# sparcityeu/SparseBase

Measured on AMD Instinct MI355X. Metric: Mrows/s, RCM reorder + CSR permute, 100M-nnz power-law (RMAT) CSR, higher is better.
Workload: dtype int32

## Files before the change

sparsebase_amd/csrc/sbx_countsort.h:

```cpp
#pragma once
#include "sbx_device.h"
#include "sbx_internal.h"
#include <utility>

namespace sbx_cs {
namespace {

constexpr int ROUNDS = 4;
constexpr int TILE = 256 * ROUNDS;
constexpr int64_t MAX_PAIRS = (int64_t)1 << 20;

template <int BITS>
__device__ __forceinline__ unsigned long long peers_of(unsigned d, bool valid) {
  unsigned long long peers = __ballot(valid);
#pragma unroll
  for (int b = 0; b < BITS; b++) {
    const bool bit = (d >> b) & 1u;
    const unsigned long long m = __ballot(bit);
    peers &= bit ? m : ~m;
  }
  return peers;
}

template <int BITS>
// ... 67 lines not shown
                                                  Emit emit) {
  constexpr int BINS = 1 << BITS, PER = BINS / 256;
  __shared__ unsigned s_scan[8];
  __shared__ unsigned s_wave[4][BINS];
  const int lane = sbx_lane(), wv = sbx_wave_in_block();
  const int64_t j0 = (int64_t)blockIdx.x * TILE + wv * (64 * ROUNDS) + lane;
  unsigned kk[ROUNDS], vv[ROUNDS];
#pragma unroll
  for (int r = 0; r < ROUNDS; r++) {
    const int64_t j = j0 + r * 64;
    kk[r] = key[j < n ? j : n - 1];
    vv[r] = val[j < n ? j : n - 1];
  }
  unsigned tt[PER], oo[PER], tsum = 0;
#pragma unroll
  for (int k = 0; k < PER; k++) {
    tt[k] = total[PER * threadIdx.x + k];
    oo[k] = off[(int64_t)(PER * threadIdx.x + k) * n_tiles + blockIdx.x];
    tsum += tt[k];
  }
#pragma unroll
  for (int w = 0; w < 4; w++)
#pragma unroll
    for (int k = 0; k < PER; k++) s_wave[w][PER * threadIdx.x + k] = 0;
  unsigned tot;
  const unsigned dbase = sbx_block_exclusive_sum<unsigned, 256>(tsum, s_scan, &tot);
  unsigned loc[ROUNDS];
#pragma unroll
  for (int r = 0; r < ROUNDS; r++) {
    const bool valid = j0 + r * 64 < n;
    const unsigned d = (kk[r] >> shift) & mask;
    const unsigned long long peers = peers_of<BITS>(d, valid);
    const unsigned rank = (unsigned)__popcll(peers & sbx_lanemask_lt());
    unsigned first = 0;
    if (valid && rank == 0) first = atomicAdd(&s_wave[wv][d], (unsigned)__popcll(peers));
    first = (unsigned)__shfl((int)first, valid ? (int)__builtin_ctzll(peers) : 0, 64);
    loc[r] = first + rank;
  }
  __syncthreads();
  {
    unsigned before = dbase;
#pragma unroll
    for (int k = 0; k < PER; k++) {
      unsigned run = before + oo[k];
#pragma unroll
      for (int w = 0; w < 4; w++) {
        const unsigned c = s_wave[w][PER * threadIdx.x + k];
        s_wave[w][PER * threadIdx.x + k] = run;
        run += c;
      }
      before += tt[k];
    }
  }
  __syncthreads();
#pragma unroll
  for (int r = 0; r < ROUNDS; r++) {
    if (j0 + r * 64 < n) {
      const unsigned d = (kk[r] >> shift) & mask;
      const unsigned pos = s_wave[wv][d] + loc[r];
      if (last) {
        emit(pos, kk[r], vv[r]);
      } else {
        key_out[pos] = kk[r];
        val_out[pos] = vv[r];
      }
    }
  }
}

static inline size_t scratch_words(int64_t n) { return (size_t)((n + TILE - 1) / TILE) * 512 + 512; }
template <int BITS, typename Emit>
static int digit_pass(sbx_handle_t h, int kid, const uint32_t *ka, const uint32_t *va, uint32_t *kb, uint32_t *vb, int64_t n,
                      int shift, int width, int last, unsigned *scratch, Emit emit) {
  constexpr int BINS = 1 << BITS;
  const int64_t n_tiles = (n + TILE - 1) / TILE;
  unsigned *total = scratch, *cnt = scratch + BINS;
  const unsigned mask = (1u << width) - 1u;
  SBX_KLAUNCH(h, kid, k_cs_count<BITS>, dim3((unsigned)n_tiles), dim3(256), ka, n, n_tiles, shift, mask, cnt);
  SBX_KLAUNCH(h, kid, k_cs_scan, dim3(BINS), dim3(256), cnt, n_tiles, total);
  SBX_KLAUNCH(h, kid, (k_cs_place<BITS, Emit>), dim3((unsigned)n_tiles), dim3(256), ka, va, n, n_tiles, (const unsigned *)cnt,
              (const unsigned *)total, shift, mask, kb, vb, last, emit);
  return SBX_OK;
}
template <typename Emit>
static int sort_emit(sbx_handle_t h, int kid, uint32_t *ka, uint32_t *va, uint32_t *kb, uint32_t *vb, int64_t n, int bits,
                     Emit emit, unsigned *scratch = nullptr) {
  if (!scratch) SBX_TRY(sbx_salloc(h, scratch_words(n), &scratch));
  if (bits < 1) bits = 1;
  const int np = (bits + 8) / 9;
  for (int p = 0, shift = 0; p < np; p++) {
    const int width = (bits - shift + (np - p) - 1) / (np - p);
    const int last = p == np - 1 ? 1 : 0;
    SBX_TRY((digit_pass<9, Emit>(h, kid, ka, va, kb, vb, n, shift, width, last, scratch, emit)));
    std::swap(ka, kb);
    std::swap(va, vb);
    shift += width;
  }
  SBX_LAUNCH_CHECK(h);
  return SBX_OK;
}

}
}
```

sparsebase_amd/csrc/sbx_rcm.hip:

```cpp
#include "sbx_device.h"
#include "sbx_internal.h"
#include "sbx_countsort.h"

#include <utility>
#include <algorithm>
#include <vector>
#include <functional>
#include <string>

namespace {

typedef int32_t I;
#ifdef SBX_RCM_I64
typedef int64_t X;
#define SBX_RCM_IT SBX_I64
#define SBX_RCM_ENTRY sbx_rcm_reorder_x64
#else
typedef int32_t X;
#define SBX_RCM_IT SBX_I32
#define SBX_RCM_ENTRY sbx_rcm_reorder_x32
#endif
constexpr int RCM_SMALL = 64;
constexpr int RCM_MID = 2048;
constexpr int RCM_MID_BATCH = 64;
// ... 974 lines not shown
                                                    RcmDev *__restrict__ dv) {
  int64_t j = (int64_t)blockIdx.x * blockDim.x + threadIdx.x;
  const int64_t stride = (int64_t)gridDim.x * blockDim.x;
  for (; j < nf; j += stride) {
    const uint32_t lo = (uint32_t)key[j];
    const I v = (I)(CM ? dorder[lo] : lo);
    q_level[j] = v;
    if (set_bits) atomicOr(&vbits[v >> 5], 1u << (v & 31));
    if (mark_frontier) {
      if (set_bits) atomicOr(&fbits[v >> 5], 1u << (v & 31));
      lpos[v] = (unsigned)j;
    }
  }
  if (blockIdx.x == 0 && threadIdx.x == 0) {
    dv->nf = 0;
    dv->n_heavy = 0;
    dv->hub_overflow = 0;
    dv->fedges = 0;
  }
}

__global__ __launch_bounds__(256) void k_visited_from_ppos(const unsigned *__restrict__ ppos,
                                                           unsigned long long *__restrict__ vbits64,
                                                           unsigned long long *__restrict__ fbits64, int64_t n) {
  const int64_t wave = ((int64_t)blockIdx.x * blockDim.x + threadIdx.x) >> 6;
  const int64_t nwaves = ((int64_t)gridDim.x * blockDim.x) >> 6;
  const int lane = sbx_lane();
  for (int64_t base = wave * 64; base < n; base += nwaves * 64) {
    const int64_t v = base + lane;
    const bool seen = v < n && ppos[v] != UNSEEN;
    const unsigned long long now = __ballot(seen);
    if (lane == 0) {
      const unsigned long long before = vbits64[base >> 6];
      vbits64[base >> 6] = now;
      if (fbits64) fbits64[base >> 6] = now & ~before;
    }
  }
}

constexpr int RCM_FW_WORDS = 64;
constexpr int RCM_FW_INLINE = 4096;

__global__ __launch_bounds__(256) void k_fresh_words(const unsigned *__restrict__ ppos,
                                                     unsigned long long *__restrict__ vbits64,
                                                     unsigned long long *__restrict__ fbits64,
                                                     unsigned long long *__restrict__ fresh64, int *__restrict__ cnt,
                                                     int *__restrict__ btot, int64_t n) {
  constexpr int WPW = RCM_FW_WORDS / 4;
  __shared__ int s_tot;
  __shared__ unsigned long long s_now[4][WPW];
  if (threadIdx.x == 0) s_tot = 0;
  __syncthreads();
  const int lane = sbx_lane(), wv = threadIdx.x >> 6;
  const int64_t w0 = (int64_t)blockIdx.x * RCM_FW_WORDS + (int64_t)wv * WPW;
  unsigned pv[WPW];
#pragma unroll
  for (int i = 0; i < WPW; i++) {
    const int64_t v = (w0 + i) * 64 + lane;
    pv[i] = v < n ? ppos[v] : UNSEEN;
  }
#pragma unroll
  for (int i = 0; i < WPW; i++) {
    const unsigned long long now = __ballot(pv[i] != UNSEEN);
    if (lane == 0) s_now[wv][i] = now;
  }
  __builtin_amdgcn_wave_barrier();
  int mine = 0;
  if (lane < WPW && (w0 + lane) * 64 < n) {
    const int64_t w = w0 + lane;
    const unsigned long long now = s_now[wv][lane];
    const unsigned long long fresh = now & ~vbits64[w];
    vbits64[w] = now;
    if (fbits64) fbits64[w] = fresh;
    fresh64[w] = fresh;
    mine = __popcll(fresh);
    cnt[w] = mine;
  }
  mine = sbx_wave_sum(mine);
  if (lane == 0 && mine) atomicAdd(&s_tot, mine);
  __syncthreads();
  if (threadIdx.x == 0) btot[blockIdx.x] = s_tot;
}

__global__ __launch_bounds__(256) void k_fresh_words_ranked(const unsigned *__restrict__ ppos,
                                                            const unsigned *__restrict__ vbits,
                                                            const uint32_t *__restrict__ dorder,
                                                            unsigned long long *__restrict__ fresh64,
                                                            int *__restrict__ cnt, int *__restrict__ btot,
                                                            int64_t n_ranked) {
  constexpr int WPW = RCM_FW_WORDS / 4;
  __shared__ int s_tot;
  if (threadIdx.x == 0) s_tot = 0;
  __syncthreads();
  const int lane = sbx_lane(), wv = threadIdx.x >> 6;
  const int64_t w0 = (int64_t)blockIdx.x * RCM_FW_WORDS + (int64_t)wv * WPW;
  uint32_t vv[WPW];
#pragma unroll
  for (int i = 0; i < WPW; i++) {
    const int64_t k = (w0 + i) * 64 + lane;
    vv[i] = dorder[k < n_ranked ? k : n_ranked - 1];
  }
  unsigned pv[WPW], vw[WPW];
#pragma unroll
  for (int i = 0; i < WPW; i++) pv[i] = ppos[vv[i]], vw[i] = vbits[vv[i] >> 5];
  int mine = 0;
#pragma unroll
  for (int i = 0; i < WPW; i++) {
    const int64_t k = (w0 + i) * 64 + lane;
    const bool fresh = k < n_ranked && pv[i] != UNSEEN && !((vw[i] >> (vv[i] & 31)) & 1u);
    const unsigned long long f = __ballot(fresh);
    if (lane == 0 && (w0 + i) * 64 < n_ranked) {
      fresh64[w0 + i] = f;
      cnt[w0 + i] = __popcll(f);
      mine += __popcll(f);
    }
  }
  if (lane == 0 && mine) atomicAdd(&s_tot, mine);
  __syncthreads();
  if (threadIdx.x == 0) btot[blockIdx.x] = s_tot;
}

__global__ __launch_bounds__(256) void k_keys_from_fresh(unsigned long long *__restrict__ fresh64,
                                                         const int *__restrict__ cnt, const int *__restrict__ btot,
                                                         int btot_is_scanned, const unsigned *__restrict__ ppos,
                                                         const uint32_t *__restrict__ dorder,
                                                         uint64_t *__restrict__ key, uint32_t *__restrict__ key32,
                                                         uint32_t *__restrict__ val32, int64_t words,
                                                         RcmDev *__restrict__ dv) {
  constexpr int WPW = RCM_FW_WORDS / 4;
  const int lane = sbx_lane(), wv = threadIdx.x >> 6;
  if (blockIdx.x == 0 && threadIdx.x == 0) reset_level_counters(dv);
  int base = 0;
  if (btot_is_scanned) {
    base = btot[blockIdx.x];
  } else {
    for (int i = lane; i < (int)blockIdx.x; i += 64) base += btot[i];
    base = sbx_wave_sum(base);
  }
  const int64_t wb = (int64_t)blockIdx.x * RCM_FW_WORDS;
  const int c = wb + lane < words ? cnt[wb + lane] : 0;
  const int inc = sbx_wave_inclusive_sum(c);
  const int excl = base + inc - c;
  const bool own = lane >= wv * WPW && lane < (wv + 1) * WPW && wb + lane < words;
  const unsigned long long mine = own ? fresh64[wb + lane] : 0ull;
  if (key32 && mine) fresh64[wb + lane] = 0;
  uint32_t vtx[WPW], low[WPW];
  int at[WPW];
  unsigned long long onmask = 0;
#pragma unroll
  for (int i = 0; i < WPW; i++) {
    const int src = wv * WPW + i;
    const unsigned long long f = __shfl(mine, src, 64);
    const int o = __shfl(excl, src, 64);
    const bool on = (f >> lane) & 1ull;
    low[i] = (uint32_t)((wb + src) * 64 + lane);
    at[i] = o + __popcll(f & sbx_lanemask_lt());
    if (on) onmask |= 1ull << i;
    vtx[i] = (on && dorder) ? dorder[low[i]] : low[i];
  }
  unsigned pp[WPW];
#pragma unroll
  for (int i = 0; i < WPW; i++) pp[i] = ((onmask >> i) & 1ull) ? ppos[vtx[i]] : 0u;
#pragma unroll
  for (int i = 0; i < WPW; i++) {
    if ((onmask >> i) & 1ull) {
      if (key32) {
        key32[at[i]] = pp[i];
        val32[at[i]] = low[i];
      } else {
        key[at[i]] = ((uint64_t)pp[i] << 32) | (uint64_t)low[i];
      }
    }
  }
}

__global__ __launch_bounds__(256) void k_rank_scatter(const I *__restrict__ nf_list, unsigned nf,
                                                      const uint32_t *__restrict__ drank,
                                                      unsigned long long *__restrict__ fresh64) {
  int64_t j = (int64_t)blockIdx.x * blockDim.x + threadIdx.x;
  const int64_t stride = (int64_t)gridDim.x * blockDim.x;
  for (; j < nf; j += stride) {
    const I v = nf_list[j];
    const uint32_t k = drank ? drank[v] : (uint32_t)v;
    atomicOr(&fresh64[k >> 6], 1ull << (k & 63));
  }
}
__global__ __launch_bounds__(64) void k_rank_counts(const unsigned long long *__restrict__ fresh64, int *__restrict__ cnt,
                                                    int *__restrict__ btot, int64_t words) {
  const int64_t w = (int64_t)blockIdx.x * RCM_FW_WORDS + threadIdx.x;
  const int c = w < words ? __popcll(fresh64[w]) : 0;
  if (w < words) cnt[w] = c;
  const int t = sbx_wave_sum(c);
  if (threadIdx.x == 0) btot[blockIdx.x] = t;
}

struct LevelEmit {
  const uint32_t *map;
  I *out;
  unsigned *bits_a, *bits_b, *pos_of;
  __device__ void operator()(unsigned pos, uint32_t, uint32_t val) const {
    const uint32_t v = map ? map[val] : val;
    out[pos] = (I)v;
    if (bits_a) atomicOr(&bits_a[v >> 5], 1u << (v & 31));
    if (bits_b) atomicOr(&bits_b[v >> 5], 1u << (v & 31));
    if (pos_of) pos_of[v] = pos;
  }
};

constexpr int RCM_BR_MAX = 48;
template <bool CM>
__global__ __launch_bounds__(1024) void k_level_sort_small(const I *__restrict__ nf_list, unsigned nf,
                                                           const unsigned *__restrict__ ppos,
                                                           const uint32_t *__restrict__ drank,
                                                           const uint32_t *__restrict__ dorder,
                                                           I *__restrict__ q_level, unsigned *__restrict__ vbits,
                                                           unsigned *__restrict__ fbits, unsigned *__restrict__ lpos,
                                                           int mark_frontier, RcmDev *__restrict__ dv) {
  constexpr int IPT = RCM_LDS_SORT / 1024;
  __shared__ uint64_t s_key[RCM_LDS_SORT];
  __shared__ uint64_t s_tmp[RCM_LDS_SORT];
  __shared__ unsigned s_end[RCM_LDS_SORT];
  __shared__ uint64_t s_mn[16], s_mx[16];
  __shared__ unsigned s_wsum[16], s_big;
  const int lane = sbx_lane(), wv = threadIdx.x >> 6;
  uint64_t mk[IPT];
  uint64_t mn = ~0ull, mx = 0;
#pragma unroll
  for (int i = 0; i < IPT; i++) {
    const unsigned j = threadIdx.x + i * 1024;
    mk[i] = ~0ull;
    if (j < nf) {
      const I v = nf_list[j];
      mk[i] = ((uint64_t)ppos[v] << 32) | (uint64_t)(CM ? drank[v] : (uint32_t)v);
      mn = mk[i] < mn ? mk[i] : mn;
      mx = mk[i] > mx ? mk[i] : mx;
    }
    s_end[j] = 0;
  }
  mn = sbx_wave_min(mn);
  mx = sbx_wave_max(mx);
  if (lane == 0) {
    s_mn[wv] = mn;
    s_mx[wv] = mx;
  }
  if (threadIdx.x == 0) s_big = 0;
  __syncthreads();
#pragma unroll
  for (int i = 0; i < 16; i++) {
    mn = s_mn[i] < mn ? s_mn[i] : mn;
    mx = s_mx[i] > mx ? s_mx[i] : mx;
  }
  const uint64_t range = mx - mn;
  int shift = 0;
  while (shift < 64 && (range >> shift) >= (uint64_t)RCM_LDS_SORT) shift++;
  unsigned bk[IPT];
#pragma unroll
  for (int i = 0; i < IPT; i++) {
    bk[i] = 0;
    if (threadIdx.x + i * 1024 < nf) {
      bk[i] = (unsigned)((mk[i] - mn) >> shift);
      atomicAdd(&s_end[bk[i]], 1u);
    }
  }
  __syncthreads();
  {
    const uint4 c = *(const uint4 *)&s_end[threadIdx.x * IPT];
    const unsigned big = c.x > c.y ? (c.x > c.z ? (c.x > c.w ? c.x : c.w) : (c.z > c.w ? c.z : c.w))
                                   : (c.y > c.z ? (c.y > c.w ? c.y : c.w) : (c.z > c.w ? c.z : c.w));
    if (big > (unsigned)RCM_BR_MAX) s_big = 1;
    const unsigned tsum = c.x + c.y + c.z + c.w;
    const unsigned inc = sbx_wave_inclusive_sum(tsum);
    if (lane == 63) s_wsum[wv] = inc;
    __syncthreads();
    unsigned base = inc - tsum;
#pragma unroll
    for (int i = 0; i < 16; i++)
      if (i < wv) base += s_wsum[i];
    uint4 e;
    e.x = base + c.x;
    e.y = e.x + c.y;
    e.z = e.y + c.z;
    e.w = e.z + c.w;
    *(uint4 *)&s_end[threadIdx.x * IPT] = e;
  }
  __syncthreads();
  if (!s_big) {
#pragma unroll
    for (int i = 0; i < IPT; i++)
      if (threadIdx.x + i * 1024 < nf) s_tmp[atomicSub(&s_end[bk[i]], 1u) - 1u] = mk[i];
    __syncthreads();
// ... 351 lines not shown
    const unsigned noff = off + fsize;
    for (unsigned j = tid; j < nf; j += 1024) {
      const uint32_t lo = (uint32_t)s_key[j];
      const I v = (I)(CM ? dorder[lo] : lo);
      q[noff + j] = v;
      atomicOr(&vbits[v >> 5], 1u << (v & 31));
      if (j < (unsigned)SL_MAXF) s_front[j] = v;
    }
    off = noff;
    fsize = nf;
    total += nf;
    level++;
    carried = true;
    __syncthreads();
  }
  ordered_edges = sbx_block_sum<unsigned long long, 1024>(ordered_edges, s_deg);
  if (tid == 0) {
    dv->sl_off = off;
    dv->sl_fsize = fsize;
    dv->sl_level = level;
    dv->sl_total = total;
    dv->sl_status = status;
    dv->sl_edges = ordered_edges;
    if (status != SL_STOP_EXPANDED) {
      dv->nf = 0;
      dv->n_heavy = 0;
      dv->hub_overflow = 0;
    }
    atomicAdd(&dv->edges, scanned);
  }
}

__global__ __launch_bounds__(256) void k_mark_frontier(const I *__restrict__ frontier, unsigned fsize,
                                                       unsigned *__restrict__ fbits, unsigned *__restrict__ lpos) {
  for (unsigned j = blockIdx.x * blockDim.x + threadIdx.x; j < fsize; j += gridDim.x * blockDim.x) {
    const I v = frontier[j];
    atomicOr(&fbits[v >> 5], 1u << (v & 31));
    lpos[v] = j;
  }
}

__global__ __launch_bounds__(256) void k_pick_root(const X *__restrict__ rp, const I *__restrict__ level,
                                                   unsigned lsize, RcmDev *__restrict__ dv) {
  int64_t j = (int64_t)blockIdx.x * blockDim.x + threadIdx.x;
  const int64_t stride = (int64_t)gridDim.x * blockDim.x;
  unsigned long long best = ~0ull;
  for (; j < lsize; j += stride) {
    const I w = level[j];
    const unsigned long long k = ((unsigned long long)(unsigned)(rp[w + 1] - rp[w]) << 32) | (unsigned)j;
    best = k < best ? k : best;
  }
  best = sbx_wave_min(best);
  if (sbx_lane() == 0 && best != ~0ull) atomicMin(&dv->best, best);
}

__global__ void k_set_root_from_best(const I *__restrict__ level, RcmDev *__restrict__ dv) {
  dv->root = (unsigned)level[(unsigned)dv->best];
}

__global__ __launch_bounds__(256) void k_reset_visited(const I *__restrict__ q, unsigned cnt, unsigned *ppos) {
  int64_t j = (int64_t)blockIdx.x * blockDim.x + threadIdx.x;
  const int64_t stride = (int64_t)gridDim.x * blockDim.x;
  for (; j < cnt; j += stride) ppos[q[j]] = UNSEEN;
}

__global__ __launch_bounds__(256) void k_comp_info(const I *__restrict__ roots, unsigned cnt, const I *__restrict__ csize,
                                                   const I *__restrict__ cbase, I *__restrict__ sizes,
                                                   I *__restrict__ bases) {
  const unsigned c = blockIdx.x * blockDim.x + threadIdx.x;
  if (c >= cnt) return;
  sizes[c] = csize[roots[c]];
  bases[c] = cbase[roots[c]];
}

__global__ __launch_bounds__(256) void k_write_component(const I *__restrict__ q, unsigned cnt, I base,
                                                         X *__restrict__ inv, const I *__restrict__ base_dev) {
  if (base_dev) base = *base_dev;
  int64_t j = (int64_t)blockIdx.x * blockDim.x + threadIdx.x;
  const int64_t stride = (int64_t)gridDim.x * blockDim.x;
  for (; j < cnt; j += stride) inv[q[j]] = base + (I)(cnt - 1 - j);
}

constexpr int64_t RCM_COUNT_SORT_MAX = (int64_t)1 << 20;

struct BfsBuffers {
  bool *claim_clean;
  const X *rp, *col;
  unsigned *vbits, *fbits, *lpos, *ppos;
  const I *label;
  int64_t nnz;
  I *q;
  I *nf_list;
  uint64_t *heavy;
  uint64_t heavy_cap;
  uint2 *hub_dir;
  uint64_t *ka, *kb;
  unsigned long long *fresh64;
  int *wcnt, *woff;
  unsigned *cs_scratch;
  const uint32_t *drank, *dorder;
  int64_t n_ranked;
  RcmDev *dv;
  int64_t n;
  unsigned max_deg;
  RcmDev *late_counts;
  bool *late_counts_ready;
  std::function<int()> *after_first_launch;
  bool hook_wants_long_cover;
  bool head_chain;
  bool *tie_unverified;
  const int *side_stage;
  hipEvent_t side_event;
  bool *side_joined;
  RcmDev *last_read;
  bool *last_read_joined;
};

static int bfs_first_launch(const BfsBuffers &b, int cover_us = 1000) {
  if (!b.after_first_launch) return SBX_OK;
  if (b.hook_wants_long_cover && cover_us < 100) return SBX_OK;
  return (*b.after_first_launch)();
}

struct BfsResult {
  unsigned count;
  unsigned levels;
  unsigned last_offset;
  unsigned last_size;
};

template <bool CM>
int run_bfs(sbx_handle_t h, const BfsBuffers &b, I fixed_root, I comp_label, BfsResult *out, bool *spec_failed = nullptr) {
  if (spec_failed) *spec_failed = false;
  const size_t bm_bytes = (size_t)((b.n + 31) / 32) * sizeof(unsigned);
  const StartClear sc = {b.vbits, (unsigned long long)((b.fbits - b.vbits) + bm_bytes / sizeof(unsigned)),
                         (unsigned *)b.fresh64, (unsigned long long)(2 * ((b.n + 63) / 64 + 1)), nullptr, 0};
  if (CM && b.side_stage && *b.side_stage >= 2 && !*b.side_joined) {
    SBX_HIP(h, hipStreamWaitEvent(h->stream, b.side_event, 0));
    *b.side_joined = true;
  }
  SBX_KLAUNCH(h, SBX_K_RCM_MISC, k_bfs_start, dim3(RCM_START_GRID), dim3(256), b.rp, b.vbits, b.fbits, b.lpos, b.ppos, b.q,
              b.dv, fixed_root, sc);
  unsigned off = 0, fsize = 1, level = 0, total = 1;
  const unsigned max_grid = (unsigned)h->num_cus * 8;
  static int heavy_per_cu = 0;
  if (heavy_per_cu == 0) {
    int nb = 0;
    if (hipOccupancyMaxActiveBlocksPerMultiprocessor(&nb, k_bfs_expand_heavy<0>, 256, 0) != hipSuccess || nb < 1) nb = 4;
    heavy_per_cu = nb;
  }
  const unsigned heavy_grid = (unsigned)h->num_cus * (unsigned)heavy_per_cu;
  int64_t remaining = b.nnz;
  int64_t frontier_edges = -1;
  bool try_small = true;
  bool frontier_unmarked = false;
  while (true) {
    bool expanded_by_small = false;
    RcmDev hd;
    if (try_small && fsize <= (unsigned)SL_MAXF) {
      SBX_KLAUNCH(h, SBX_K_BFS_SMALL, (k_bfs_small_levels<CM>), dim3(1), dim3(1024), b.rp, b.col, b.q, b.vbits, b.fbits,
                  b.lpos, b.ppos, b.nf_list, b.drank, b.dorder, off, fsize, level, total, b.dv);
      SBX_LAUNCH_CHECK(h);
      SBX_TRY(bfs_first_launch(b));
      SBX_TRY(sbx_readback(h, &hd, b.dv, sizeof(RcmDev)));
      if (b.tie_unverified && *b.tie_unverified) {
        *b.tie_unverified = false;
// ... 20 lines not shown
      expanded_by_small = true;
    }
    try_small = true;
    if (!expanded_by_small) {
    const bool bottom_up = frontier_edges >= 0 && fsize >= 8192 && (double)frontier_edges > sbx_sw().bu_ratio * (double)remaining;
    if (bottom_up) {
      if (frontier_unmarked) {
        SBX_HIP(h, hipMemsetAsync(b.fbits, 0, bm_bytes, h->stream));
        SBX_KLAUNCH(h, SBX_K_RCM_MISC, k_mark_frontier, dim3(sbx_grid_for(fsize, 256, 1024)), dim3(256),
                    (const I *)(b.q + off), fsize, b.fbits, b.lpos);
      }
      SBX_KLAUNCH(h, SBX_K_BFS_BOTTOMUP, k_bfs_bottom_up, dim3(max_grid), dim3(256), b.rp, b.col, b.label, comp_label,
                  (const unsigned *)b.vbits, (const unsigned *)b.fbits, (const unsigned *)b.lpos, b.ppos, b.nf_list,
                  b.n, b.dv, b.heavy, b.heavy_cap);
      if (b.max_deg > (unsigned)RCM_BU_HEAVY)
        SBX_KLAUNCH(h, SBX_K_BFS_BOTTOMUP, k_bfs_bottom_up_heavy, dim3(8 * (unsigned)h->num_cus), dim3(256), b.rp, b.col,
                    (const unsigned *)b.fbits, (const unsigned *)b.lpos, b.ppos, b.nf_list, b.dv,
                    (const uint64_t *)b.heavy, b.heavy_cap);
    } else {
      const unsigned waves_needed = (fsize + RCM_VPW - 1) / RCM_VPW;
      unsigned grid = (waves_needed + 3) / 4;
      if (grid > max_grid) grid = max_grid;
      if (grid < 1) grid = 1;
      const UnorderedSweep none = {nullptr, nullptr, nullptr, 0u};
      const bool split = b.max_deg > (unsigned)RCM_LIGHT && fsize >= 4096 && !h->prof_on && sbx_sw().rcm_split_expand && h->aux_ready;
      if (split) {
        hipStream_t main_s = h->stream;
        const bool was_dirty = h->aux_dirty;
        SBX_KLAUNCH(h, SBX_K_BFS_EXPAND, k_bfs_expand<0>, dim3(grid), dim3(256), b.rp, b.col, (const I *)(b.q + off),
                    fsize, level + 1, (const unsigned *)b.vbits, b.ppos, b.nf_list, b.heavy, b.hub_dir, b.dv, none, 1);
        SBX_HIP(h, hipEventRecord(h->aux_event[4], main_s));
        SBX_HIP(h, hipStreamWaitEvent(h->aux_stream[2], h->aux_event[4], 0));
        h->aux_dirty = true;
        h->stream = h->aux_stream[2];
        hipLaunchKernelGGL(k_bfs_expand<0>, dim3(grid), dim3(256), 0, h->stream, b.rp, b.col, (const I *)(b.q + off), fsize,
                           level + 1, (const unsigned *)b.vbits, b.ppos, b.nf_list, b.heavy, b.hub_dir, b.dv, none, 2);
        const hipError_t e1 = hipGetLastError(), e2 = hipEventRecord(h->aux_event[5], h->stream);
        h->stream = main_s;
        if (e1 != hipSuccess || e2 != hipSuccess) SBX_FAIL(h, SBX_ERR_HIP, "run_bfs: side launch failed");
        SBX_KLAUNCH(h, SBX_K_BFS_HEAVY, k_bfs_expand_heavy<0>, dim3(heavy_grid), dim3(256), b.rp, b.col,
                    (const I *)(b.q + off), level + 1, (const unsigned *)b.vbits, b.ppos, b.nf_list,
                    (const uint64_t *)b.heavy, (const uint2 *)b.hub_dir, grid, b.dv, none);
        SBX_HIP(h, hipStreamWaitEvent(main_s, h->aux_event[5], 0));
        h->aux_dirty = was_dirty;
      } else {
      SBX_KLAUNCH(h, SBX_K_BFS_EXPAND, k_bfs_expand<0>, dim3(grid), dim3(256), b.rp, b.col, (const I *)(b.q + off),
                  fsize, level + 1, (const unsigned *)b.vbits, b.ppos, b.nf_list, b.heavy, b.hub_dir, b.dv, none, 0);
      if (b.max_deg > (unsigned)RCM_LIGHT)
        SBX_KLAUNCH(h, SBX_K_BFS_HEAVY, k_bfs_expand_heavy<0>, dim3(heavy_grid), dim3(256), b.rp, b.col,
                    (const I *)(b.q + off), level + 1, (const unsigned *)b.vbits, b.ppos, b.nf_list,
                    (const uint64_t *)b.heavy, (const uint2 *)b.hub_dir, grid, b.dv, none);
      }
    }
    SBX_LAUNCH_CHECK(h);
    SBX_TRY(bfs_first_launch(b));
    SBX_TRY(sbx_readback(h, &hd, b.dv, sizeof(RcmDev)));
    if (b.last_read) *b.last_read = hd, *b.last_read_joined = b.side_joined && *b.side_joined;
    }
    frontier_unmarked = false;
    const unsigned nf = hd.nf;
    if (SBX_DEBUG_RCM_LEVELS)
      fprintf(stderr, "[rcm %s] level %u: frontier %u vertices / %lld edges, unvisited edges %lld -> %u new vertices / %llu edges\n",
              CM ? "cm" : "plain", level, fsize, (long long)frontier_edges, (long long)remaining, nf,
              (unsigned long long)hd.fedges);
    if (nf == 0) break;
    if (frontier_edges < 0) remaining -= (int64_t)0;
    frontier_edges = (int64_t)hd.fedges;
    remaining -= frontier_edges;
    if (remaining < 0) remaining = 0;
    I *q_next = b.q + off + fsize;
    const bool next_bottom_up = nf >= 8192 && (double)frontier_edges > sbx_sw().bu_ratio * (double)remaining;
    const int mark_frontier = next_bottom_up ? 1 : 0;
    const bool bitmap_pass = nf > (unsigned)RCM_LDS_SORT && (int64_t)nf >= std::max<int64_t>(RCM_REBUILD_BITS, b.n / 128);
    if (mark_frontier && !bitmap_pass) SBX_HIP(h, hipMemsetAsync(b.fbits, 0, bm_bytes, h->stream));
    if (nf <= RCM_LDS_SORT) {
      SBX_KLAUNCH(h, SBX_K_LEVEL_ORDER, (k_level_sort_small<CM>), dim3(1), dim3(1024), (const I *)b.nf_list, nf,
                  (const unsigned *)b.ppos, b.drank, b.dorder, q_next, b.vbits, b.fbits, b.lpos, mark_frontier, b.dv);
    } else {
      const unsigned g = sbx_grid_for(nf, 256, 4096);
      const int set_bits = bitmap_pass ? 0 : 1;
      sbx_radix_pass passes[16];
      int np;
      int low_bits = 32;
      if (sbx_sw().rcm_count_sort && (int64_t)nf <= RCM_COUNT_SORT_MAX) {
        const int64_t span = CM ? b.n_ranked : b.n;
        const int64_t words = (span + 63) / 64;
        const int64_t fw_blocks = (words + RCM_FW_WORDS - 1) / RCM_FW_WORDS;
        if (!CM && !set_bits) {
          SBX_KLAUNCH(h, SBX_K_LEVEL_ORDER, k_fresh_words, dim3((unsigned)fw_blocks), dim3(256), (const unsigned *)b.ppos,
                      (unsigned long long *)b.vbits,
                      mark_frontier ? (unsigned long long *)b.fbits : (unsigned long long *)nullptr, b.fresh64, b.wcnt,
                      b.woff, b.n);
        } else if (CM && (int64_t)nf * 16 >= b.n_ranked) {
          SBX_KLAUNCH(h, SBX_K_LEVEL_ORDER, k_fresh_words_ranked, dim3((unsigned)fw_blocks), dim3(256),
                      (const unsigned *)b.ppos, (const unsigned *)b.vbits, b.dorder, b.fresh64, b.wcnt, b.woff, b.n_ranked);
        } else {
          SBX_KLAUNCH(h, SBX_K_LEVEL_ORDER, k_rank_scatter, dim3(g), dim3(256), (const I *)b.nf_list, nf,
                      CM ? b.drank : (const uint32_t *)nullptr, b.fresh64);
          SBX_KLAUNCH(h, SBX_K_LEVEL_ORDER, k_rank_counts, dim3((unsigned)fw_blocks), dim3(64),
                      (const unsigned long long *)b.fresh64, b.wcnt, b.woff, words);
        }
        const int scanned = fw_blocks > RCM_FW_INLINE ? 1 : 0;
        if (scanned) SBX_TRY(sbx_exclusive_scan_i32(h, b.woff, b.woff, fw_blocks, nullptr));
        uint32_t *k32 = (uint32_t *)b.ka, *v32 = k32 + b.n, *k32b = (uint32_t *)b.kb, *v32b = k32b + b.n;
        SBX_KLAUNCH(h, SBX_K_LEVEL_ORDER, k_keys_from_fresh, dim3((unsigned)fw_blocks), dim3(256), b.fresh64,
                    (const int *)b.wcnt, (const int *)b.woff, scanned, (const unsigned *)b.ppos,
                    CM ? b.dorder : (const uint32_t *)nullptr, (uint64_t *)nullptr, k32, v32, words, b.dv);
        const LevelEmit em = {CM ? b.dorder : nullptr, q_next, set_bits ? b.vbits : nullptr,
                              (set_bits && mark_frontier) ? b.fbits : nullptr, mark_frontier ? b.lpos : nullptr};
        SBX_TRY(sbx_cs::sort_emit(h, SBX_K_LEVEL_ORDER, k32, v32, k32b, v32b, (int64_t)nf,
                                  sbx_bits_for((uint64_t)(fsize - 1)), em, b.cs_scratch));
        np = -1;
      } else if (!CM && !set_bits) {
        const int64_t words = (b.n + 63) / 64;
        const int64_t fw_blocks = (words + RCM_FW_WORDS - 1) / RCM_FW_WORDS;
        SBX_KLAUNCH(h, SBX_K_LEVEL_ORDER, k_fresh_words, dim3((unsigned)fw_blocks), dim3(256), (const unsigned *)b.ppos,
                    (unsigned long long *)b.vbits,
                    mark_frontier ? (unsigned long long *)b.fbits : (unsigned long long *)nullptr, b.fresh64, b.wcnt,
                    b.woff, b.n);
        const int scanned = fw_blocks > RCM_FW_INLINE ? 1 : 0;
        if (scanned) SBX_TRY(sbx_exclusive_scan_i32(h, b.woff, b.woff, fw_blocks, nullptr));
        SBX_KLAUNCH(h, SBX_K_LEVEL_ORDER, k_keys_from_fresh, dim3((unsigned)fw_blocks), dim3(256),
                    b.fresh64, (const int *)b.wcnt, (const int *)b.woff, scanned,
                    (const unsigned *)b.ppos, (const uint32_t *)nullptr, b.ka, (uint32_t *)nullptr, (uint32_t *)nullptr, words,
                    b.dv);
        np = sbx_radix_plan(0, 0, 32, 32 + sbx_bits_for((uint64_t)(fsize - 1)), passes);
      } else if (CM && !set_bits && sbx_sw().rcm_ranked_keys && (int64_t)nf * sbx_sw().rcm_ranked_div >= b.n_ranked) {
        const int64_t words = (b.n_ranked + 63) / 64;
        const int64_t fw_blocks = (words + RCM_FW_WORDS - 1) / RCM_FW_WORDS;
        SBX_KLAUNCH(h, SBX_K_LEVEL_ORDER, k_fresh_words_ranked, dim3((unsigned)fw_blocks), dim3(256),
                    (const unsigned *)b.ppos, (const unsigned *)b.vbits, b.dorder, b.fresh64, b.wcnt, b.woff, b.n_ranked);
        const int scanned = fw_blocks > RCM_FW_INLINE ? 1 : 0;
        if (scanned) SBX_TRY(sbx_exclusive_scan_i32(h, b.woff, b.woff, fw_blocks, nullptr));
        SBX_KLAUNCH(h, SBX_K_LEVEL_ORDER, k_keys_from_fresh, dim3((unsigned)fw_blocks), dim3(256),
                    b.fresh64, (const int *)b.wcnt, (const int *)b.woff, scanned,
                    (const unsigned *)b.ppos, b.dorder, b.ka, (uint32_t *)nullptr, (uint32_t *)nullptr, words, b.dv);
        np = sbx_radix_plan(0, 0, 32, 32 + sbx_bits_for((uint64_t)(fsize - 1)), passes);
      } else {
        low_bits = sbx_bits_for((uint64_t)(b.n - 1));
        SBX_KLAUNCH(h, SBX_K_LEVEL_ORDER, (k_level_keys<CM>), dim3(g), dim3(256), (const I *)b.nf_list, nf,
                    (const unsigned *)b.ppos, b.drank, b.ka, b.dv, low_bits);
        np = sbx_radix_plan(0, low_bits + sbx_bits_for((uint64_t)(fsize - 1)), 0, 0, passes);
      }
      if (np < 0) {
      } else if (np > 0) {
        const sbx_radix_emit em = {CM ? b.dorder : nullptr, (uint32_t *)q_next, set_bits ? b.vbits : nullptr,
                                   (set_bits && mark_frontier) ? b.fbits : nullptr, mark_frontier ? b.lpos : nullptr,
                                   low_bits < 32 ? (1u << low_bits) - 1u : 0u};
        SBX_TRY(sbx_radix_sort_emit(h, b.ka, b.kb, nf, passes, np, &em));
      } else {
        SBX_KLAUNCH(h, SBX_K_LEVEL_ORDER, (k_level_emit<CM>), dim3(g), dim3(256), (const uint64_t *)b.ka, nf, b.dorder,
                    q_next, b.vbits, b.fbits, b.lpos, mark_frontier, set_bits, b.dv);
      }
      if (CM && !set_bits)
        SBX_KLAUNCH(h, SBX_K_LEVEL_ORDER, k_visited_from_ppos, dim3(sbx_grid_for(b.n, 256 * 4, 4096)), dim3(256),
                    (const unsigned *)b.ppos, (unsigned long long *)b.vbits,
                    mark_frontier ? (unsigned long long *)b.fbits : (unsigned long long *)nullptr, b.n);
    }
    SBX_LAUNCH_CHECK(h);
    off += fsize;
    fsize = nf;
    total += nf;
    level++;
  }
  out->count = total;
  out->levels = level + 1;
  out->last_offset = off;
  out->last_size = fsize;
  return SBX_OK;
}


#ifndef SBX_DEBUG_UBU_RATIO
#define SBX_DEBUG_UBU_RATIO 0.5
#endif
constexpr double UBU_RATIO = SBX_DEBUG_UBU_RATIO;

#ifndef SBX_UR_GRID
#define SBX_UR_GRID 64
#endif
constexpr unsigned UR_GRID = SBX_UR_GRID;
constexpr unsigned UR_CONTINUE = 0, UR_DONE = 1, UR_STOP = 2, UR_DEEP = 3;
constexpr unsigned UR_MAX_E = 1u << 18;
constexpr unsigned UR_MAX_N = 1024;
constexpr unsigned UC_DONE = 1, UC_BU = 2, UC_SMALL = 3, UC_HOST = 4;
struct ChainInit {
  unsigned off, size, level, total;
  long long remaining;
  double bu_ratio;
};
__device__ __forceinline__ void uc_advance(RcmDev *dv, double bu_ratio) {
  const unsigned built = dv->uc_level + 1;
  const unsigned nf = __hip_atomic_load(&dv->unf[built & 1], __ATOMIC_RELAXED, __HIP_MEMORY_SCOPE_AGENT);
  const unsigned long long fe = __hip_atomic_load(&dv->ufedges[built & 1], __ATOMIC_RELAXED, __HIP_MEMORY_SCOPE_AGENT);
  if (nf == 0) {
    dv->uc_mode = UC_DONE;
    return;
  }
  long long rem = dv->uc_remaining - (long long)fe;
  if (rem < 0) rem = 0;
  dv->uc_remaining = rem;
  dv->uc_off += dv->uc_size;
  dv->uc_size = nf;
  dv->uc_total += nf;
  dv->uc_level = built;
  dv->uc_fe = fe;
  if (fe <= (unsigned long long)UR_MAX_E && nf <= UR_MAX_N) dv->uc_mode = UC_SMALL;
  else if (nf >= 1024 && (double)fe > bu_ratio * (double)rem) dv->uc_mode = UC_BU;
  else dv->uc_mode = UC_HOST;
}
__device__ __forceinline__ void uc_begin(RcmDev *dv, const ChainInit &ci) {
  dv->uc_off = ci.off, dv->uc_size = ci.size, dv->uc_level = ci.level, dv->uc_total = ci.total;
  dv->uc_remaining = ci.remaining;
  dv->uc_flips = 0;
// ... 1559 lines not shown
  SBX_TRY(sbx_salloc(h, (size_t)n, &lpos));
  const size_t heavy_cap = (size_t)(nnz / RCM_LIGHT + nnz / RCM_CHUNK + 1024);
  SBX_TRY(sbx_salloc(h, heavy_cap, &heavy));
  SBX_TRY(sbx_salloc(h, (size_t)n, &ka));
  SBX_TRY(sbx_salloc(h, (size_t)n, &kb));

  const unsigned gn = sbx_grid_for(n, 256, 8192);
  const size_t bm_bytes = (size_t)((n + 31) / 32) * sizeof(unsigned);
  unsigned *ucnt = nullptr;
  SBX_TRY(sbx_salloc(h, (size_t)DEG_UNITS * 4, &ucnt));
  SBX_KLAUNCH(h, SBX_K_RCM_MISC, k_deg_count, dim3(DEG_UNITS / 4), dim3(256), rp, n, ucnt, csize, dist, ppos);
  SBX_KLAUNCH(h, SBX_K_RCM_MISC, k_deg_reduce, dim3(1), dim3(1024), (const unsigned *)ucnt, dv);
  SBX_LAUNCH_CHECK(h);
  const bool unordered_ok = sbx_sw().rcm_unordered && h->rcm_gb_backoff == 0;
  if (h->rcm_gb_backoff > 0) h->rcm_gb_backoff--;
  const bool lazy_counts = unordered_ok && !h->prof_on && sbx_sw().rcm_overlap;
  RcmDev hd0;
  bool hd0_ready = false;
  if (!lazy_counts) {
    SBX_TRY(sbx_readback(h, &hd0, dv, sizeof(RcmDev)));
    hd0_ready = true;
  }
  int64_t n_ranked = hd0_ready ? (int64_t)hd0.n_nonempty : 0;
  const uint32_t *dorder = nullptr;
  hipStream_t main_stream = h->stream;
  const bool side = !h->prof_on && sbx_sw().rcm_overlap;
  BfsBuffers b;
  if (side) {
    SBX_TRY(sbx_aux_streams(h));
    SBX_HIP(h, hipEventRecord(h->aux_event[0], main_stream));
  }
  bool ranks_enqueued = false;
  bool cc_forked = false;
  std::function<int()> enqueue_ranks = [&]() -> int {
    if (ranks_enqueued) return SBX_OK;
    ranks_enqueued = true;
    if (side) {
      void *slot = nullptr;
      SBX_TRY(sbx_arena_alloc(h, SBX_RS_SLOT_BYTES, &slot));
      SBX_HIP(h, hipStreamWaitEvent(h->aux_stream[0], h->aux_event[0], 0));
      h->aux_dirty = true;
      h->stream = h->aux_stream[0];
      if (hipMemsetAsync(slot, 0, SBX_RS_SLOT_BYTES, h->stream) != hipSuccess) {
        h->stream = main_stream;
        SBX_FAIL(h, SBX_ERR_HIP, "sbx_rcm_reorder: hipMemsetAsync failed");
      }
      h->rs_override = slot;
    }
    int rc = SBX_OK;
    rc = sbx_degree_ranks(h, SBX_RCM_IT, rp, n, (int64_t)hd0.n_nonempty, (int64_t)hd0.n_top, hd0.max_deg, drank, did_a);
    dorder = did_a;
    b.dorder = dorder;
    if (side && rc == SBX_OK && hipEventRecord(h->aux_event[1], h->stream) != hipSuccess) rc = SBX_ERR_HIP;
    h->stream = main_stream;
    h->rs_override = nullptr;
    return rc;
  };
  if (!side) SBX_TRY(enqueue_ranks());
  bool ranks_joined = !side;
  auto join_ranks = [&]() -> int {
    if (!ranks_enqueued) SBX_TRY(enqueue_ranks());
    if (!ranks_joined) {
      SBX_HIP(h, hipStreamWaitEvent(main_stream, h->aux_event[1], 0));
      ranks_joined = true;
      if (!cc_forked) h->aux_dirty = false;
    }
    return SBX_OK;
  };
  bool claim_clean = false;
  b.claim_clean = &claim_clean;
  b.after_first_launch = &enqueue_ranks;
  b.hook_wants_long_cover = true;
  b.head_chain = true;
  bool tie_unverified = false;
  b.tie_unverified = &tie_unverified;
  b.side_stage = nullptr, b.side_event = nullptr, b.side_joined = nullptr, b.last_read = nullptr, b.last_read_joined = nullptr;
  b.rp = rp; b.col = col; b.vbits = vbits; b.fbits = fbits; b.lpos = lpos; b.ppos = ppos; b.label = nullptr;
  b.nnz = nnz; b.q = q; b.nf_list = nf_list; b.heavy = heavy; b.heavy_cap = heavy_cap;
  SBX_TRY(sbx_salloc(h, (size_t)std::max<int64_t>((int64_t)h->num_cus * 8, RCM_DIR_MAX), &b.hub_dir));
  b.ka = ka; b.kb = kb; b.drank = drank; b.dorder = dorder; b.n_ranked = n_ranked; b.dv = dv; b.n = n;
  SBX_TRY(sbx_salloc(h, (size_t)(n + 63) / 64 + 1, &b.fresh64));
  SBX_TRY(sbx_salloc(h, (size_t)(n + 63) / 64 + 1, &b.wcnt));
  SBX_TRY(sbx_salloc(h, (size_t)(n + 63) / 64 / RCM_FW_WORDS + 2, &b.woff));
  SBX_TRY(sbx_salloc(h, sbx_cs::scratch_words(std::min<int64_t>(n, RCM_COUNT_SORT_MAX)), &b.cs_scratch));
  b.max_deg = hd0_ready ? hd0.max_deg : 0u;
  b.late_counts = hd0_ready ? nullptr : &hd0;
  b.late_counts_ready = &hd0_ready;
  BfsResult r0;
  r0.count = 0;
  unsigned char *claim8 = nullptr;
  unsigned *cone = nullptr, *nbits = nullptr;
  SBX_TRY(sbx_salloc(h, (size_t)n + 64, &claim8));
  SBX_TRY(sbx_salloc(h, (size_t)(bm_bytes / sizeof(unsigned)) + 2, &nbits));
  SBX_TRY(sbx_salloc(h, (size_t)(bm_bytes / sizeof(unsigned)) + 2, &cone));
  bool r0_unordered = false;
  bool deep0 = true;
  int64_t unordered_sweeps = 0;
  if (!hd0_ready) {
    SBX_TRY(run_ubfs(h, b, claim8, nbits, cone, (I)-1, (I)-1, &r0, &deep0));
    if (!hd0_ready) SBX_FAIL(h, SBX_ERR_INTERNAL, "sbx_rcm_reorder: the first sweep returned without a read-back");
    n_ranked = (int64_t)hd0.n_nonempty;
    b.n_ranked = n_ranked;
    b.max_deg = hd0.max_deg;
    b.late_counts = nullptr;
  }
  if (hd0_ready && lazy_counts) b.head_chain = false;
  const I v0 = hd0.first_vertex == UNSEEN ? (I)-1 : (I)hd0.first_vertex;
  if (v0 < 0) {
    r0.count = 0;
    deep0 = true;
    SBX_HIP(h, hipMemsetAsync(cbits, 0, bm_bytes, h->stream));
  }
  if (v0 >= 0) {
    bool deep = deep0;
    if (!lazy_counts && unordered_ok) SBX_TRY(run_ubfs(h, b, claim8, nbits, cone, v0, (I)-1, &r0, &deep));
    b.head_chain = false;
    r0_unordered = !deep;
    unordered_sweeps += r0_unordered;
    if (deep) SBX_TRY(run_bfs<false>(h, b, v0, (I)-1, &r0));
    SBX_KLAUNCH(h, SBX_K_RCM_MISC, k_copy_words, dim3(sbx_grid_for((int64_t)(bm_bytes / sizeof(unsigned)), 256, 1024)),
                dim3(256), cbits, (const unsigned *)vbits, (int64_t)(bm_bytes / sizeof(unsigned)));
    SBX_LAUNCH_CHECK(h);
  }
  struct Searched {
    BfsResult r;
    int64_t sweeps, levels, candidate;
    bool cm_done;
  };
  Searched sd0;
  bool comp0_searched = false, small_on_side = false;
  auto search_component = [&](I root, I size, bool have_first_sweep, Searched &out) -> int {
    BfsResult &r = out.r;
    int64_t prev_ecc = -1, ecc = 0;
    int64_t &sweeps = out.sweeps, &levels = out.levels, &candidate = out.candidate;
    sweeps = levels = candidate = 0;
    I fixed = root;
    bool &cm_done = out.cm_done;
    cm_done = false;
    bool deep = !unordered_ok;
    while (prev_ecc != ecc) {
      prev_ecc = ecc;
      bool unordered = false;
      if (have_first_sweep) {
        r = r0;
        have_first_sweep = false;
        unordered = r0_unordered;
        if (!unordered) deep = true;
      } else {
        auto settle_tie = [&]() -> int {
          bool ab = false;
          SBX_TRY(ubfs_pick_root_slow(h, b, cone, r, &ab, true));
          if (ab) {
            deep = true;
            SBX_TRY(run_bfs<false>(h, b, -1, root, &r));
            SBX_KLAUNCH(h, SBX_K_RCM_MISC, k_pick_root, dim3(sbx_grid_for(r.last_size, 256, 1024)), dim3(256), rp,
                        (const I *)(q + r.last_offset), r.last_size, dv);
            SBX_KLAUNCH(h, SBX_K_RCM_MISC, k_set_root_from_best, dim3(1), dim3(1), (const I *)(q + r.last_offset), dv);
            SBX_TRY(reset_ppos(h, (const I *)q, r.count, ppos, n));
          }
          return SBX_OK;
        };
        if (candidate >= RCM_SPECULATE_FROM) {
          SBX_TRY(join_ranks());
          bool sf = false;
          SBX_TRY(run_bfs<true>(h, b, fixed, root, &r, &sf));
          if (sf) {
            SBX_TRY(settle_tie());
// ... 256 lines not shown
```

Before: 1339.

## Fuse first count-sort digit histogram into fresh-word scan for large RCM levels

For large Cuthill-McKee levels where the frontier covers a big share of ranked vertices, the fresh-word kernel now also builds the first radix digit histogram. A new placement kernel scatters fresh vertices straight from the bitmap into the first digit's buckets, so the separate key-build and first count pass are skipped. The counting-sort path is also extended to frontiers far larger than the old 1M cap, replacing the generic radix sort there. Count-sort scratch is now sized to n, which uses more memory, and the bucket grid is now tied to bitmap word blocks instead of key tiles.

```diff
diff --git a/sparsebase_amd/csrc/sbx_countsort.h b/sparsebase_amd/csrc/sbx_countsort.h
--- a/sparsebase_amd/csrc/sbx_countsort.h
+++ b/sparsebase_amd/csrc/sbx_countsort.h
@@ -173,14 +173,26 @@
               (const unsigned *)total, shift, mask, kb, vb, last, emit);
   return SBX_OK;
 }
+static inline int digit_count(int bits) { return ((bits < 1 ? 1 : bits) + 8) / 9; }
+static inline int digit_width(int bits, int p) {
+  if (bits < 1) bits = 1;
+  const int np = digit_count(bits);
+  int shift = 0, width = 0;
+  for (int i = 0; i <= p; i++) {
+    width = (bits - shift + (np - i) - 1) / (np - i);
+    shift += width;
+  }
+  return width;
+}
 template <typename Emit>
-static int sort_emit(sbx_handle_t h, int kid, uint32_t *ka, uint32_t *va, uint32_t *kb, uint32_t *vb, int64_t n, int bits,
-                     Emit emit, unsigned *scratch = nullptr) {
-  if (!scratch) SBX_TRY(sbx_salloc(h, scratch_words(n), &scratch));
+static int sort_emit_from(sbx_handle_t h, int kid, uint32_t *ka, uint32_t *va, uint32_t *kb, uint32_t *vb, int64_t n,
+                          int bits, int first, Emit emit, unsigned *scratch) {
   if (bits < 1) bits = 1;
-  const int np = (bits + 8) / 9;
-  for (int p = 0, shift = 0; p < np; p++) {
-    const int width = (bits - shift + (np - p) - 1) / (np - p);
+  const int np = digit_count(bits);
+  int shift = 0;
+  for (int p = 0; p < first; p++) shift += digit_width(bits, p);
+  for (int p = first; p < np; p++) {
+    const int width = digit_width(bits, p);
     const int last = p == np - 1 ? 1 : 0;
     SBX_TRY((digit_pass<9, Emit>(h, kid, ka, va, kb, vb, n, shift, width, last, scratch, emit)));
     std::swap(ka, kb);
@@ -190,6 +202,12 @@
   SBX_LAUNCH_CHECK(h);
   return SBX_OK;
 }
-
-}
-}
+template <typename Emit>
+static int sort_emit(sbx_handle_t h, int kid, uint32_t *ka, uint32_t *va, uint32_t *kb, uint32_t *vb, int64_t n, int bits,
+                     Emit emit, unsigned *scratch = nullptr) {
+  if (!scratch) SBX_TRY(sbx_salloc(h, scratch_words(n), &scratch));
+  return sort_emit_from(h, kid, ka, va, kb, vb, n, bits, 0, emit, scratch);
+}
+
+}
+}
diff --git a/sparsebase_amd/csrc/sbx_rcm.hip b/sparsebase_amd/csrc/sbx_rcm.hip
--- a/sparsebase_amd/csrc/sbx_rcm.hip
+++ b/sparsebase_amd/csrc/sbx_rcm.hip
@@ -1080,15 +1080,20 @@
   if (threadIdx.x == 0) btot[blockIdx.x] = s_tot;
 }
 
+template <bool COUNT>
 __global__ __launch_bounds__(256) void k_fresh_words_ranked(const unsigned *__restrict__ ppos,
                                                             const unsigned *__restrict__ vbits,
                                                             const uint32_t *__restrict__ dorder,
                                                             unsigned long long *__restrict__ fresh64,
                                                             int *__restrict__ cnt, int *__restrict__ btot,
-                                                            int64_t n_ranked) {
+                                                            int64_t n_ranked, unsigned mask,
+                                                            unsigned *__restrict__ dcnt) {
   constexpr int WPW = RCM_FW_WORDS / 4;
+  constexpr int BINS = COUNT ? 512 : 1;
   __shared__ int s_tot;
+  __shared__ unsigned s_hist[BINS];
   if (threadIdx.x == 0) s_tot = 0;
+  if (COUNT) s_hist[threadIdx.x] = 0, s_hist[threadIdx.x + 256] = 0;
   __syncthreads();
   const int lane = sbx_lane(), wv = threadIdx.x >> 6;
   const int64_t w0 = (int64_t)blockIdx.x * RCM_FW_WORDS + (int64_t)wv * WPW;
@@ -1109,9 +1114,20 @@
     const unsigned long long f = __ballot(fresh);
     if (lane == 0 && (w0 + i) * 64 < n_ranked) {
       fresh64[w0 + i] = f;
-      cnt[w0 + i] = __popcll(f);
+      if (!COUNT) cnt[w0 + i] = __popcll(f);
       mine += __popcll(f);
     }
+    if (COUNT && f) {
+      const unsigned d = pv[i] & mask;
+      const unsigned long long peers = sbx_cs::peers_of<9>(d, fresh);
+      if (fresh && (peers & sbx_lanemask_lt()) == 0) atomicAdd(&s_hist[d], (unsigned)__popcll(peers));
+    }
+  }
+  if (COUNT) {
+    __syncthreads();
+    dcnt[(int64_t)threadIdx.x * gridDim.x + blockIdx.x] = s_hist[threadIdx.x];
+    dcnt[(int64_t)(threadIdx.x + 256) * gridDim.x + blockIdx.x] = s_hist[threadIdx.x + 256];
+    return;
   }
   if (lane == 0 && mine) atomicAdd(&s_tot, mine);
   __syncthreads();
@@ -1204,6 +1220,87 @@
     if (pos_of) pos_of[v] = pos;
   }
 };
+
+template <typename Emit>
+__global__ __launch_bounds__(256) void k_level_place_fresh(unsigned long long *__restrict__ fresh64, int64_t words,
+                                                           const unsigned *__restrict__ ppos,
+                                                           const uint32_t *__restrict__ dorder,
+                                                           const unsigned *__restrict__ off,
+                                                           const unsigned *__restrict__ total, unsigned mask,
+                                                           uint32_t *__restrict__ key_out, uint32_t *__restrict__ val_out,
+                                                           int last, Emit emit, RcmDev *__restrict__ dv) {
+  constexpr int WPW = RCM_FW_WORDS / 4, BINS = 512, PER = BINS / 256;
+  __shared__ unsigned s_scan[8];
+  __shared__ unsigned s_wave[4][BINS];
+  const int lane = sbx_lane(), wv = threadIdx.x >> 6;
+  if (blockIdx.x == 0 && threadIdx.x == 0) reset_level_counters(dv);
+  const int64_t w0 = (int64_t)blockIdx.x * RCM_FW_WORDS + (int64_t)wv * WPW;
+  const unsigned long long mine = lane < WPW && w0 + lane < words ? fresh64[w0 + lane] : 0ull;
+  if (mine) fresh64[w0 + lane] = 0;
+  unsigned tt[PER], oo[PER], tsum = 0;
+#pragma unroll
+  for (int k = 0; k < PER; k++) {
+    tt[k] = total[PER * threadIdx.x + k];
+    oo[k] = off[(int64_t)(PER * threadIdx.x + k) * gridDim.x + blockIdx.x];
+    tsum += tt[k];
+  }
+#pragma unroll
+  for (int w = 0; w < 4; w++)
+#pragma unroll
+    for (int k = 0; k < PER; k++) s_wave[w][PER * threadIdx.x + k] = 0;
+  unsigned pp[WPW];
+  unsigned long long onmask = 0;
+#pragma unroll
+  for (int i = 0; i < WPW; i++) {
+    const unsigned long long f = __shfl(mine, i, 64);
+    if ((f >> lane) & 1ull) onmask |= 1ull << i;
+    pp[i] = ((onmask >> i) & 1ull) ? dorder[(w0 + i) * 64 + lane] : 0u;
+  }
+#pragma unroll
+  for (int i = 0; i < WPW; i++) pp[i] = ((onmask >> i) & 1ull) ? ppos[pp[i]] : 0u;
+  unsigned tot;
+  const unsigned dbase = sbx_block_exclusive_sum<unsigned, 256>(tsum, s_scan, &tot);
+  unsigned loc[WPW];
+#pragma unroll
+  for (int i = 0; i < WPW; i++) {
+    const bool on = (onmask >> i) & 1ull;
+    const unsigned long long peers = sbx_cs::peers_of<9>(pp[i] & mask, on);
+    const unsigned rank = (unsigned)__popcll(peers & sbx_lanemask_lt());
+    unsigned first = 0;
+    if (on && rank == 0) first = atomicAdd(&s_wave[wv][pp[i] & mask], (unsigned)__popcll(peers));
+    first = (unsigned)__shfl((int)first, on ? (int)__builtin_ctzll(peers) : 0, 64);
+    loc[i] = first + rank;
+  }
+  __syncthreads();
+  {
+    unsigned before = dbase;
+#pragma unroll
+    for (int k = 0; k < PER; k++) {
+      unsigned run = before + oo[k];
+#pragma unroll
+      for (int w = 0; w < 4; w++) {
+        const unsigned c = s_wave[w][PER * threadIdx.x + k];
+        s_wave[w][PER * threadIdx.x + k] = run;
+        run += c;
+      }
+      before += tt[k];
+    }
+  }
+  __syncthreads();
+#pragma unroll
+  for (int i = 0; i < WPW; i++) {
+    if ((onmask >> i) & 1ull) {
+      const unsigned pos = s_wave[wv][pp[i] & mask] + loc[i];
+      const uint32_t rk = (uint32_t)((w0 + i) * 64 + lane);
+      if (last) {
+        emit(pos, pp[i], rk);
+      } else {
+        key_out[pos] = pp[i];
+        val_out[pos] = rk;
+      }
+    }
+  }
+}
 
 constexpr int RCM_BR_MAX = 48;
 template <bool CM>
@@ -1721,6 +1818,10 @@
 }
 
 constexpr int64_t RCM_COUNT_SORT_MAX = (int64_t)1 << 20;
+#ifndef SBX_RCM_FRESH_SORT_MAX
+#define SBX_RCM_FRESH_SORT_MAX ((int64_t)1 << 31)
+#endif
+constexpr int64_t RCM_FRESH_SORT_MAX = SBX_RCM_FRESH_SORT_MAX;
 
 struct BfsBuffers {
   bool *claim_clean;
@@ -1907,7 +2008,28 @@
       sbx_radix_pass passes[16];
       int np;
       int low_bits = 32;
-      if (sbx_sw().rcm_count_sort && (int64_t)nf <= RCM_COUNT_SORT_MAX) {
+      const bool gathered = CM && (int64_t)nf * 16 >= b.n_ranked;
+      if (sbx_sw().rcm_count_sort && gathered && (int64_t)nf <= RCM_FRESH_SORT_MAX) {
+        const int64_t words = (b.n_ranked + 63) / 64;
+        const int64_t fw_blocks = (words + RCM_FW_WORDS - 1) / RCM_FW_WORDS;
+        const int bits = sbx_bits_for((uint64_t)(fsize - 1));
+        const unsigned mask0 = (1u << sbx_cs::digit_width(bits, 0)) - 1u;
+        const int last = sbx_cs::digit_count(bits) == 1 ? 1 : 0;
+        unsigned *total = b.cs_scratch, *dcnt = b.cs_scratch + 512;
+        uint32_t *k32 = (uint32_t *)b.ka, *v32 = k32 + b.n, *k32b = (uint32_t *)b.kb, *v32b = k32b + b.n;
+        const LevelEmit em = {b.dorder, q_next, set_bits ? b.vbits : nullptr,
+                              (set_bits && mark_frontier) ? b.fbits : nullptr, mark_frontier ? b.lpos : nullptr};
+        SBX_KLAUNCH(h, SBX_K_LEVEL_ORDER, k_fresh_words_ranked<true>, dim3((unsigned)fw_blocks), dim3(256),
+                    (const unsigned *)b.ppos, (const unsigned *)b.vbits, b.dorder, b.fresh64, (int *)nullptr,
+                    (int *)nullptr, b.n_ranked, mask0, dcnt);
+        SBX_KLAUNCH(h, SBX_K_LEVEL_ORDER, sbx_cs::k_cs_scan, dim3(512), dim3(256), dcnt, fw_blocks, total);
+        SBX_KLAUNCH(h, SBX_K_LEVEL_ORDER, k_level_place_fresh<LevelEmit>, dim3((unsigned)fw_blocks), dim3(256), b.fresh64,
+                    words, (const unsigned *)b.ppos, b.dorder, (const unsigned *)dcnt, (const unsigned *)total, mask0,
+                    k32, v32, last, em, b.dv);
+        if (!last) SBX_TRY(sbx_cs::sort_emit_from(h, SBX_K_LEVEL_ORDER, k32, v32, k32b, v32b, (int64_t)nf, bits, 1, em,
+                                                  b.cs_scratch));
+        np = -1;
+      } else if (sbx_sw().rcm_count_sort && (int64_t)nf <= RCM_COUNT_SORT_MAX) {
         const int64_t span = CM ? b.n_ranked : b.n;
         const int64_t words = (span + 63) / 64;
         const int64_t fw_blocks = (words + RCM_FW_WORDS - 1) / RCM_FW_WORDS;
@@ -1916,9 +2038,10 @@
                       (unsigned long long *)b.vbits,
                       mark_frontier ? (unsigned long long *)b.fbits : (unsigned long long *)nullptr, b.fresh64, b.wcnt,
                       b.woff, b.n);
-        } else if (CM && (int64_t)nf * 16 >= b.n_ranked) {
-          SBX_KLAUNCH(h, SBX_K_LEVEL_ORDER, k_fresh_words_ranked, dim3((unsigned)fw_blocks), dim3(256),
-                      (const unsigned *)b.ppos, (const unsigned *)b.vbits, b.dorder, b.fresh64, b.wcnt, b.woff, b.n_ranked);
+        } else if (gathered) {
+          SBX_KLAUNCH(h, SBX_K_LEVEL_ORDER, k_fresh_words_ranked<false>, dim3((unsigned)fw_blocks), dim3(256),
+                      (const unsigned *)b.ppos, (const unsigned *)b.vbits, b.dorder, b.fresh64, b.wcnt, b.woff, b.n_ranked,
+                      0u, (unsigned *)nullptr);
         } else {
           SBX_KLAUNCH(h, SBX_K_LEVEL_ORDER, k_rank_scatter, dim3(g), dim3(256), (const I *)b.nf_list, nf,
                       CM ? b.drank : (const uint32_t *)nullptr, b.fresh64);
@@ -1953,8 +2076,9 @@
       } else if (CM && !set_bits && sbx_sw().rcm_ranked_keys && (int64_t)nf * sbx_sw().rcm_ranked_div >= b.n_ranked) {
         const int64_t words = (b.n_ranked + 63) / 64;
         const int64_t fw_blocks = (words + RCM_FW_WORDS - 1) / RCM_FW_WORDS;
-        SBX_KLAUNCH(h, SBX_K_LEVEL_ORDER, k_fresh_words_ranked, dim3((unsigned)fw_blocks), dim3(256),
-                    (const unsigned *)b.ppos, (const unsigned *)b.vbits, b.dorder, b.fresh64, b.wcnt, b.woff, b.n_ranked);
+        SBX_KLAUNCH(h, SBX_K_LEVEL_ORDER, k_fresh_words_ranked<false>, dim3((unsigned)fw_blocks), dim3(256),
+                    (const unsigned *)b.ppos, (const unsigned *)b.vbits, b.dorder, b.fresh64, b.wcnt, b.woff, b.n_ranked,
+                    0u, (unsigned *)nullptr);
         const int scanned = fw_blocks > RCM_FW_INLINE ? 1 : 0;
         if (scanned) SBX_TRY(sbx_exclusive_scan_i32(h, b.woff, b.woff, fw_blocks, nullptr));
         SBX_KLAUNCH(h, SBX_K_LEVEL_ORDER, k_keys_from_fresh, dim3((unsigned)fw_blocks), dim3(256),
@@ -3680,7 +3804,7 @@
   SBX_TRY(sbx_salloc(h, (size_t)(n + 63) / 64 + 1, &b.fresh64));
   SBX_TRY(sbx_salloc(h, (size_t)(n + 63) / 64 + 1, &b.wcnt));
   SBX_TRY(sbx_salloc(h, (size_t)(n + 63) / 64 / RCM_FW_WORDS + 2, &b.woff));
-  SBX_TRY(sbx_salloc(h, sbx_cs::scratch_words(std::min<int64_t>(n, RCM_COUNT_SORT_MAX)), &b.cs_scratch));
+  SBX_TRY(sbx_salloc(h, sbx_cs::scratch_words(n), &b.cs_scratch));
   b.max_deg = hd0_ready ? hd0.max_deg : 0u;
   b.late_counts = hd0_ready ? nullptr : &hd0;
   b.late_counts_ready = &hd0_ready;
```

Result: no change. 1347, median of 6 (+0.6%).
